# retinal-information-processing-lab/gaussian_processes

Hardware: AMD Instinct MI355X
Metric: GP fits/sec (kernel+chol+solve+grad loglik) at N=8192 d=256 (higher is better)
Workload: dtype f64; 1 GPU; N=8192 d=256 single cell f64, one M-step closure evaluation with 6 gradients (BASELINE configs[2], headline); N=8192, d=256, parallelism=independent units over 1 GPU(s), one process per GPU, no data-path collective

## Files before the change

### gaussian_processes_amd/_lib.py

```python
from __future__ import annotations

import ctypes
import os

from .build import lib_path

vp, i32, i64, f64 = ctypes.c_void_p, ctypes.c_int, ctypes.c_int64, ctypes.c_double
pd = ctypes.POINTER(ctypes.c_double)



class DevGemmArgs(ctypes.Structure):
    _fields_ = ([(n, vp) for n in ("A", "B", "C")] + [(n, i64) for n in ("lda", "ldb", "ldc", "sA", "sB", "sC")] +
                [("alpha", f64), ("beta", f64)] +
                [(n, vp) for n in ("sk_ws", "aux", "sumsq", "Ap", "Bp", "Cp", "auxp", "sumsqp")] +
                [(n, ctypes.c_int32) for n in ("M", "N", "K", "a_kmajor", "b_kmajor", "out_lower", "a_tri", "b_tri", "batch",
                                               "split_k", "tile", "walk", "epi", "nptr", "k_slabs")])


class DevGemmRoute(ctypes.Structure):
    _fields_ = [(n, ctypes.c_int32) for n in ("rc", "tile", "sk_first", "xcd", "stages", "half_occ", "edge", "epi",
                                              "sumsq_entries", "blocks", "pair", "slabs")]


_SIGS = {
    "gpfit_version": (i32, []),
    "gpfit_last_error": (ctypes.c_char_p, []),
    "gpfit_dgemm": (i32, [vp, i32, i32, i32, i32, i32, f64, vp, i64, vp, i64, f64, vp, i64, i32, i32, i32]),
    "gpfit_dgemm_ex": (i32, [vp, i32, i32, i32, i32, i32, f64, vp, i64, vp, i64, f64, vp, i64, i32, i32, i32, i32, i32]),
    "gpfit_ctx_create": (i32, [i32, i64, i64, i64, ctypes.POINTER(vp)]),
    "gpfit_ctx_destroy": (None, [vp]),
    "gpfit_check_limits": (i32, [pd, pd, pd]),
    "gpfit_localker_mask": (i32, [pd, i32, i32, vp, ctypes.POINTER(i64)]),
    "gpfit_localker": (i32, [vp, vp, pd, i32, i32, vp, i64, vp, vp]),
    "gpfit_acosker": (i32, [vp, vp, f64, vp, i64, i64, vp, i64, i64, i64, vp, i64, vp, vp, i64, vp]),
    "gpfit_acosker_pullback": (i32, [vp, vp, f64, vp, i64, i64, vp, i64, i64, i64, vp, i64, vp, i64, vp, vp, i64, pd]),
    "gpfit_acosker_diag": (i32, [vp, vp, f64, vp, i64, i64, i64, vp, i64, vp, vp, vp]),
# ... 83 lines not shown
```

### gaussian_processes_amd/csrc/api_dev.hip

```cpp
#include "gemm_core.h"
#include "context.h"
#include "gpfit_mi355x.h"

#include <cstring>

namespace gpfit {
namespace {

template <typename R>
int fill(const gpfit_dev_gemm_args& d, GemmArgsT<R>& g) {
  g = GemmArgsT<R>{};
  g.A = (const R*)d.A; g.B = (const R*)d.B; g.C = (R*)d.C;
  g.lda = d.lda; g.ldb = d.ldb; g.ldc = d.ldc;
  g.M = d.M; g.N = d.N; g.K = d.K;
  g.alpha = d.alpha; g.beta = d.beta;
  g.a_kmajor = d.a_kmajor; g.b_kmajor = d.b_kmajor;
  g.out_lower = d.out_lower; g.a_tri = d.a_tri; g.b_tri = d.b_tri;
  g.batch = d.batch > 0 ? d.batch : 1;
  g.sA = d.sA; g.sB = d.sB; g.sC = d.sC;
  g.split_k = d.split_k > 0 ? d.split_k : 1;
  g.k_slabs = d.k_slabs > 0 ? d.k_slabs : 0;
  g.tile = d.tile;
  g.reverse = d.walk & 15;
  g.half_occ = (d.walk >> 4) & 1;
  g.sk_ws = d.sk_ws;
  g.epi = d.epi;
  g.aux = (R*)d.aux;
  g.sumsq = d.sumsq;
  g.nptr = d.nptr;
  if (d.nptr < 0 || d.nptr > GEMM_MAXB) return d.nptr < 0 ? -3 : 0;
  for (int b = 0; b < d.nptr; ++b) {
    if (!d.Ap || !d.Bp || !d.Cp) return -3;
    g.Ap[b] = (const R*)d.Ap[b];
    g.Bp[b] = (const R*)d.Bp[b];
    g.Cp[b] = (R*)d.Cp[b];
    g.auxp[b] = d.auxp ? (R*)d.auxp[b] : nullptr;
    g.sumsqp[b] = d.sumsqp ? d.sumsqp[b] : nullptr;
  }
  return 0;
}

template <typename R>
int route(const gpfit_dev_gemm_args& d, const gpfit_dev_gemm_args* d2, gpfit_dev_gemm_route_t& o) {
  std::memset(&o, 0, sizeof(o));
  o.sk_first = -1;
  GemmArgsT<R> a, b;
  if (fill(d, a) != 0 || (d2 && fill(*d2, b) != 0)) return -3;
  GemmRoute r = d2 ? gemm_pair_shape(a, b) : gemm_route(a);
  long blocks = d2 ? r.tiles : -1;
  if (r.rc == 0 && r.sched == GEMM_STREAMK) {
    SkHostPlan plan;
    if (streamk_plan_host(a, r.sk_first, plan) != 0) r.stay_data_parallel();
    else blocks = plan.blocks;
  }
  if (r.rc == 0 && r.sched == GEMM_XCD) {
    std::vector<int> table;
    if (xcd_plan_host(a, table) != 0) return -3;
    r.gx = (int)table.size();
  }
  o.rc = r.rc; o.tile = r.tile; o.sk_first = r.sk_first; o.xcd = r.sched == GEMM_XCD; o.stages = r.stages;
  o.half_occ = r.half; o.edge = r.edge; o.epi = r.epi; o.sumsq_entries = r.sumsq_entries; o.slabs = r.slabs;
  o.pair = d2 && r.rc == 0;
  o.blocks = (int)std::min<long>(blocks >= 0 ? blocks : (long)r.gx * r.gy * r.gz, 0x7fffffffL);
  return 0;
}

template <typename R>
int64_t plan(const gpfit_dev_gemm_args& d, int kind, int32_t* out, int64_t cap) {
  GemmArgsT<R> a;
  if (fill(d, a) != 0 || a.M <= 0 || a.N <= 0) return -3;
  const GemmRoute r = gemm_route(a);
  if (r.rc != 0) return -3;
  if (kind == 1) {
    if (r.sched != GEMM_XCD) return -1;
    std::vector<int> table;
    if (xcd_plan_host(a, table) != 0) return -1;
// ... 112 lines not shown
```

### gaussian_processes_amd/csrc/common.h

```cpp
#pragma once
#include <hip/hip_runtime.h>
#include <stdint.h>
#include <stdio.h>
#include <string>

namespace gpfit {

constexpr double PI32 = 3.1415927410125732;

constexpr int TILE = 128;
constexpr int TRMV_ROWS = 128;
constexpr int KTILE = 16;

void set_error(const std::string& msg);

#define GP_HIP(expr)                                                                     \
  do {                                                                                   \
    hipError_t _e = (expr);                                                              \
    if (_e != hipSuccess) {                                                              \
      gpfit::set_error(std::string(#expr) + ": " + hipGetErrorString(_e));               \
      return -100;                                                                       \
    }                                                                                    \
  } while (0)

// ... 14 lines not shown
  R* C;
  int64_t lda, ldb, ldc;
  int M, N, K;
  double alpha, beta;
  int a_kmajor, b_kmajor;
  int out_lower;
  int a_tri, b_tri;
  int batch;
  int64_t sA, sB, sC;
  int split_k;
  int k_slabs;
  int tile;
  int reverse;
  int half_occ;
  void* sk_ws;
  int reserved;
  const int* sched;
  int epi;
  R* aux;
  double* sumsq;
  int nptr;
  const R* Ap[GEMM_MAXB];
  const R* Bp[GEMM_MAXB];
  R* Cp[GEMM_MAXB];
  R* auxp[GEMM_MAXB];
  double* sumsqp[GEMM_MAXB];
};
using GemmArgs = GemmArgsT<double>;

constexpr int SLAB_TILE = 64;
struct SlabPlan {
  int nt, ks, live;
  int full, rb;
  int items;
};
__host__ __device__ inline SlabPlan slab_plan(int M, int slabs) {
  SlabPlan p;
  p.nt = (M + SLAB_TILE - 1) / SLAB_TILE;
  p.ks = (p.nt + slabs - 1) / slabs;
  p.live = (p.nt + p.ks - 1) / p.ks;
  p.full = p.live + p.ks * (p.live * (p.live - 1) / 2);
// ... 28 lines not shown
enum { GEMM_DATA_PARALLEL = 0, GEMM_XCD = 1, GEMM_STREAMK = 2 };
struct GemmRoute {
  int rc;
  const char* error;
  int sched;
  int sk_first;
  int tile;
  int tiles, tiles_n;
  int stages;
  int edge;
  int half;
  int gx, gy, gz;
  int epi;
  int sumsq_entries;
  int slabs;
  void stay_data_parallel() { sched = GEMM_DATA_PARALLEL; sk_first = -1; gx = tiles; }
};
template <typename R> GemmRoute gemm_route(const GemmArgsT<R>& a);
template <typename R> int gemm_pick_tile(const GemmArgsT<R>& a);
template <typename R> int launch_gemm(const GemmArgsT<R>& a, const GemmRoute& r, hipStream_t s);
template <typename R> int launch_gemm(const GemmArgsT<R>& a, hipStream_t s) { return launch_gemm(a, gemm_route(a), s); }
template <typename R> int launch_gemm_streamk(const GemmArgsT<R>& a, const GemmRoute& r, hipStream_t s);
template <typename R> int launch_gemm_xcd(const GemmArgsT<R>& a, GemmRoute r, hipStream_t s);
template <typename R> int launch_gemm_plain(const GemmArgsT<R>& a, const GemmRoute& r, hipStream_t s);
template <typename R> GemmRoute gemm_pair_shape(const GemmArgsT<R>& a, const GemmArgsT<R>& b);
template <typename R> int launch_gemm_pair(const GemmArgsT<R>& a, const GemmArgsT<R>& b, const GemmRoute& h, hipStream_t s);

template <typename R>
struct GramArgsT {
  const R* XCt;
// ... 18 lines not shown
```

### gaussian_processes_amd/csrc/fit.hip

```cpp
#include "product.h"
#include "gemm_core.h"
#include "gpfit_mi355x.h"

#include <algorithm>
#include <chrono>
#include <cmath>
#include <cstdlib>
#include <cstring>
#include <limits>

namespace gpfit {

static thread_local gpfit_ctx* g_prof = nullptr;

static int walk(Walk which) {
  static int w[W_COUNT] = {3, 2, 1, 9, 9, 2, 2};
  static bool init = false;
  if (!init) {
    init = true;
    if (const char* e = getenv("GPFIT_WALKS")) {
      int v[W_COUNT];
      if (sscanf(e, "%d,%d,%d,%d,%d,%d,%d", &v[0], &v[1], &v[2], &v[3], &v[4], &v[5], &v[6]) == 7)
        for (int i = 0; i < W_COUNT; ++i) w[i] = v[i];
    }
// ... 126 lines not shown
  const int64_t slab = (int64_t)d.M * C.ld;
  bool any = false;
  for (int i = 0; i < cnt && !off; ++i)
    any = any || (partial[i] && std::min<int64_t>(splitk_for(d.M, d.N, d.K), partial_elems[i] / std::max<int64_t>(1, slab)) > 1);
  if (!any) return product(lane, d, alpha, a, b, into(C));
  for (int i = 0; i < cnt; ++i) {
    Operand<R> ai = a, bi = b;
    ai.m.cnt = bi.m.cnt = 1;
    ai.m.p[0] = a.m.p[i]; bi.m.p[0] = b.m.p[i];
    GP_TRY(gemm_splitk(lane, d, alpha, ai, bi, C.p[i], C.ld, partial[i], partial_elems[i]));
  }
  return 0;
}

static int fused_epilogues() {
  static const int v = getenv("GPFIT_FUSED_EPI") ? atoi(getenv("GPFIT_FUSED_EPI")) : 7;
  return v;
}

template <typename R>
int product(Lane lane, Dims d, double alpha, const Operand<R>& a, const Operand<R>& b, const Output<R>& c, int walk, Epilogue<R>* e) {
  const int cnt = c.m.cnt, epi = e ? e->which : 0;
  if (e) { e->carried = false; e->sumsq_entries = 0; }
  if (cnt <= 0) return 0;
  if (cnt > GEMM_MAXB) {
    set_error("product: more problems than a pointer batch holds");
    return -3;
  }
  GemmArgsT<R> g = product_args(lane, d, alpha, a, b, c, walk);
  static const bool no_batch = getenv("GPFIT_NO_BATCH") != nullptr;
  if (cnt == 1 || gemm_pick_tile(g) == TILE || no_batch) {
    auto problem = [&](int i, bool fused) {
      g.A = a.m.p[i]; g.B = b.m.p[i]; g.C = c.m.p[i];
      g.epi = fused ? epi : 0; g.aux = fused ? e->aux[i] : nullptr; g.sumsq = fused ? e->sumsq[i] : nullptr;
    };
    GemmRoute routes[GEMM_MAXB];
    bool fused = epi != 0;
    for (int i = 0; i < cnt && fused; ++i) {
      problem(i, true);
      routes[i] = gemm_route(g);
      fused = routes[i].epi != 0;
    }
    for (int i = 0; i < cnt; ++i) {
      problem(i, fused);
      GP_TRY(fused ? run_gemm(lane.s, g, routes[i]) : run_gemm(lane.s, g));
    }
    if (e) e->carried = fused;
    if (fused) e->sumsq_entries = routes[0].sumsq_entries;
    return 0;
  }
  g = batch_args(lane, d, alpha, a, b, c, walk, e);
  GemmRoute r = gemm_route(g);
  if (epi && r.epi == 0) {
    g.epi = 0;
    r = gemm_route(g);
  }
  if (e) { e->carried = g.epi != 0; e->sumsq_entries = r.sumsq_entries; }
  return run_gemm(lane.s, g, r);
}
template int product<double>(Lane, Dims, double, const Operand<double>&, const Operand<double>&, const Output<double>&, int,
                             Epilogue<double>*);
template int product<float>(Lane, Dims, double, const Operand<float>&, const Operand<float>&, const Output<float>&, int,
                            Epilogue<float>*);

template <typename R>
int potrf_lockstep(const CholBatchT<R>& B, int r0, int n, uint32_t need, Lane lane, uint32_t halves) {
  const int64_t ld = B.ld;
  const hipStream_t s = lane.s;
  const uint32_t all = (B.nb >= 32) ? 0xffffffffu : ((1u << B.nb) - 1u);
// ... 72 lines not shown
    GP_TRY(product(lane, {n2, n1, n2}, -1.0, plain(tril(blk(need, B.Li, r1, r1))), plain(blk(need, B.Tmp, r1, r0)),
                   into(blk(need, B.Li, r1, r0)), walk(W_MERGE)));
  }
  return 0;
}

template int potrf_lockstep<double>(const CholBatchT<double>&, int, int, uint32_t, Lane, uint32_t);
template int potrf_lockstep<float>(const CholBatchT<float>&, int, int, uint32_t, Lane, uint32_t);

template <typename R>
struct TwoSidedBufs { R* Q; const R* Li; R *W, *Z, *H; const R* L; int64_t ld; int min_split; };
template <typename R, typename P>
static Mat<P> ts_blk(int cnt, const TwoSidedBufs<R>* b, const int* r0, P* TwoSidedBufs<R>::*X, int dr, int dc) {
  return mats(cnt, b[0].ld, [&](int i) { const int o = r0 ? r0[i] : 0; return b[i].*X + (int64_t)(o + dr) * b[i].ld + o + dc; });
}
template <typename R>
static int dual_update_list(Lane lane, Dims d, double alpha, const Operand<R>& a, const Operand<R>& b, const Mat<R>& H,
                            const Mat<R>& Z, int wk) {
  const int cnt = H.cnt;
  const int64_t ld = H.ld;
  Epilogue<R> e{4};
  for (int i = 0; i < cnt; ++i) e.aux[i] = Z.p[i];
  bool fused = false;
  if (fused_epilogues() & 4) {
    GemmArgsT<R> g = product_args(lane, d, alpha, a, b, into(H), wk);
    g.epi = 4; g.aux = Z.p[0];
    static const bool no_batch = getenv("GPFIT_NO_BATCH") != nullptr;
    if (cnt > 1 && gemm_pick_tile(g) != TILE && !no_batch) { g.nptr = cnt; g.batch = cnt; }
    fused = gemm_route(g).epi != 0;
  }
  if (fused) {
    GP_TRY(product(lane, d, alpha, a, b, into(H), wk, &e));
    if (!e.carried) {
      set_error("two_sided: the dual-update epilogue was announced but not carried");
      return -100;
    }
    return 0;
  }
  for (int i = 0; i < cnt; ++i)
    GP_HIP(hipMemcpy2DAsync(H.p[i], (size_t)ld * sizeof(R), Z.p[i], (size_t)ld * sizeof(R), (size_t)d.N * sizeof(R), (size_t)d.M,
                            hipMemcpyDeviceToDevice, lane.s));
  GP_TRY(product(lane, d, alpha, a, b, into(H, 1.0), wk));
  for (int i = 0; i < cnt; ++i) GP_TRY(launch_axpby_block<R>(Z.p[i], ld, H.p[i], ld, d.M, d.N, 1.0, 1.0, lane.s));
  return 0;
}

template <typename R>
static int two_sided_list(Lane lane, int cnt, const TwoSidedBufs<R>* b, const int* r0, int n) {
  if (cnt <= 0) return 0;
  using TS = TwoSidedBufs<R>;
  auto blk = [&](auto X, int dr, int dc) { return ts_blk(cnt, b, r0, X, dr, dc); };
  const int k = n / TILE;
  if (n < b[0].min_split || k < 2) {
    static const int wbase_walk = getenv("GPFIT_WBASE_WALK") ? atoi(getenv("GPFIT_WBASE_WALK")) : 0;
    GP_TRY(product(lane, {n, n, n}, 1.0, trans(blk(&TS::Q, 0, 0)), plain(tril(blk(&TS::Li, 0, 0))), into(blk(&TS::Z, 0, 0)),
                   walk(W_RBASE)));
    return product(lane, {n, n, n}, 0.5, trans(tril(blk(&TS::Li, 0, 0))), plain(blk(&TS::Z, 0, 0)),
// ... 420 lines not shown
    Epilogue<R> ep{};
    for (int q = 0; q < cnt * cb && q < GEMM_MAXB; ++q) ep.sumsq[q] = cs[q / cb]->frob_part + ent + (q % cb) * e;
    GP_TRY(normed_product({nblk, nblk, nblk}, plain(tril(blk(&PJ::Li))), plain(tril(blk(&PJ::LV))), into_lower(blk(&PJ::T)),
                          walk(W_T), ask, ep, "a diagonal block of T"));
    ent += cb * e;
    return 0;
  };
  const int r_both[2] = {0, n1};
  if (n2 == n1 && 2 * cnt <= GEMM_MAXB) GP_TRY(diag_blocks(2, r_both, n1));
  else {
    GP_TRY(diag_blocks(1, r_both, n1));
    GP_TRY(diag_blocks(1, r_both + 1, n2));
  }
  {
    auto blk = [&](auto X, int64_t o) { return mats(cnt, ld, [&](int i) { return a[i].*X + o; }); };
    for (int i = 0; i < cnt; ++i)
      GP_HIP(hipMemcpy2DAsync(a[i].Z + o21, (size_t)ld * sizeof(R), a[i].LV + o21, (size_t)ld * sizeof(R), (size_t)n1 * sizeof(R),
                              (size_t)n2, hipMemcpyDeviceToDevice, s));
    GP_TRY(product(lane, {n2, n1, n1}, -1.0, plain(blk(&PJ::L, o21)), plain(tril(blk(&PJ::T, 0))), into(blk(&PJ::Z, o21), 1.0),
                   walk(W_TMP)));
    int e = asks_21();
    const bool ask = e > 0;
    if (!ask) e = (n2 / TILE) * (n1 / TILE);
    Epilogue<R> ep{};
    for (int i = 0; i < cnt; ++i) ep.sumsq[i] = cs[i]->frob_part + ent;
    GP_TRY(normed_product({n2, n1, n2}, plain(tril(blk(&PJ::Li, o21 + n1))), plain(blk(&PJ::Z, o21)), into(blk(&PJ::T, o21)),
                          walk(W_MERGE), ask, ep, "T21"));
    ent += e;
  }
  for (int i = 0; i < cnt; ++i) {
    if (any_fused) GP_TRY(launch_frob_finish(cs[i]->frob_part, ent, cs[i]->scal + S_TRACE, s));
    else GP_TRY(launch_frob_lower(a[i].T, ld, np, cs[i]->scal + S_TRACE, cs[i]->frob_part, s));
  }
  return 0;
}
// ... 10 lines not shown
    Epilogue<R> e{(fused_epilogues() & 2) ? 2 : 0};
    for (int i = 0; i < cnt; ++i) e.sumsq[i] = cs[i]->frob_part;
    GP_TRY(product(lane, {np, np, np}, 1.0, plain(tril(all(&PJ::Li, ld))), plain(tril(all(&PJ::LV, ld))), into_lower(all(&PJ::T, ld)),
                   walk(W_T), &e));
    for (int i = 0; i < cnt; ++i) {
      if (e.carried) GP_TRY(launch_frob_finish(cs[i]->frob_part, e.sumsq_entries, cs[i]->scal + S_TRACE, s));
      else GP_TRY(launch_frob_lower(a[i].T, ld, np, cs[i]->scal + S_TRACE, cs[i]->frob_part, s));
    }
  } else {
    GP_TRY(t_in_blocks<R>(lane, cnt, cs, a, np));
  }
  phase(4, s);
  if (!want_grad) return 0;
  {
    Epilogue<R> mirror{(fused_epilogues() & 1) ? 1 : 0};
    GP_TRY(product(lane, {np, np, np}, -1.0, plain(tril(all(&PJ::T, ld))), trans(tril(all(&PJ::T, ld))), into_lower(all(&PJ::W, ld)),
                   walk(W_Q), &mirror));
    for (int i = 0; i < cnt; ++i) {
      GP_TRY(launch_add_diag(a[i].W, ld, np, 1.0, s));
      if (!mirror.carried) GP_TRY(launch_symmetrize(a[i].W, ld, np, s));
    }
  }
  phase(5, s);
  {
    static const int ts_min = getenv("GPFIT_TS_MIN") ? atoi(getenv("GPFIT_TS_MIN")) : 4096;
    TwoSidedBufs<R> tb[GEMM_MAXB];
    for (int i = 0; i < cnt; ++i)
      tb[i] = TwoSidedBufs<R>{a[i].W, a[i].Li, a[i].T, a[i].Z, a[i].H, a[i].L, ld, ts_min > 0 ? ts_min : (1 << 30)};
    if (blocks) GP_TRY(two_sided_top<R>(lane, cnt, tb, np));
    else {
      int r0[GEMM_MAXB];
      for (int i = 0; i < cnt; ++i) r0[i] = 0;
      GP_TRY(two_sided_list<R>(lane, cnt, tb, r0, np));
    }
  }
// ... 52 lines not shown
  const bool blocks = top_in_blocks(np, sizeof(R));
  c->cur_n = n; c->cur_np = np; c->cur_d = d; c->cur_dp = dp;

  ++g_eval_count;
  const auto t_host0 = std::chrono::steady_clock::now();
  auto phase = [&](int i, hipStream_t st) {
    if (c->profile != 2) return;
    if (!c->phase_ev[i]) (void)hipEventCreate(&c->phase_ev[i]);
    (void)hipEventRecord(c->phase_ev[i], st);
  };
  c->phase_valid = false;
  phase(0, s);
  const Lane lane = main_lane(c, s);
  prof_begin(c);
  struct ProfGuard { gpfit_ctx* c; ~ProfGuard() { prof_end(c); } } prof_guard{c};
  GP_HIP(hipMemsetAsync(c->info, 0, 4 * sizeof(int), s));
  GP_HIP(hipMemcpyAsync(c->pix, c->pix_host, (size_t)d * sizeof(int), hipMemcpyHostToDevice, s));
  GP_HIP(hipMemsetAsync(RP(c->mpad), 0, (size_t)np * sizeof(R), s));
  GP_HIP(hipMemcpyAsync(RP(c->mpad), m, (size_t)n * sizeof(R), hipMemcpyDeviceToDevice, s));

  const bool reuse_V = (want_grad & 2) && c->lv_valid && c->lv_n == n && c->lv_bytes == (int)sizeof(R);
  const bool async_call = (want_grad & 4) != 0;
  const bool mixed_grad = (want_grad & 8) != 0 && sizeof(R) == 8 && (want_grad & 1);
  want_grad &= 1;
  static const int side_min_env = getenv("GPFIT_SIDE_MIN") ? atoi(getenv("GPFIT_SIDE_MIN")) : 1024;
  const int side_min = async_call ? 0 : side_min_env;
  if (!async_call) GP_TRY(ensure_side_stream(c));
  c->side_ev_next = 0;
  if (!reuse_V) {
    c->lv_valid = false; c->lv32_valid = false;
    GP_HIP(hipEventRecord(c->ev_fork, s));
    GP_HIP(hipStreamWaitEvent(c->aux, c->ev_fork, 0));
    GP_TRY(launch_pack_lower(V, ldv, n, RP(c->Vbuf), ld, np, c->aux));
    GP_HIP(hipEventRecord(c->ev_join, c->aux));
  }

  GP_TRY(build_kernel<R>(c, lane, th, d, dp, n_rows, n_cols, X, ldx, n, np, 0));
  GP_TRY(launch_moments(RP(c->Kvec), RP(c->q), RP(c->Cos), ld, V, ldv, m, r, n, A, lambda0, RP(c->lam_m), RP(c->lam_var), RP(c->fvec),
                        RP(c->wl), c->scal + S_RLAM, c->sumA_part, c->info + INFO_MOMENTS, s));
  phase(1, s);
  {
    CholBatchT<R> cb;
    cb.nb = reuse_V ? 1 : 2;
    cb.A[0] = RP(c->Kbuf); cb.L[0] = RP(c->Lbuf); cb.Li[0] = RP(c->Libuf); cb.Tmp[0] = RP(c->Tmp); cb.info[0] = c->info + INFO_K;
    cb.A[1] = RP(c->Vbuf); cb.L[1] = RP(c->LVbuf); cb.Li[1] = RP(c->LiVbuf); cb.Tmp[1] = RP(c->TmpV); cb.info[1] = c->info + INFO_V;
    cb.ld = ld; cb.ctx = c; cb.side_min = side_min;
    if (!reuse_V) GP_HIP(hipStreamWaitEvent(s, c->ev_join, 0));
    if (blocks) GP_TRY(potrf_lockstep<R>(cb, 0, np, 0u, lane, 1u));
    else GP_TRY(potrf_lockstep<R>(cb, 0, np, 1u, lane));
    if (!reuse_V) GP_TRY(launch_logdet(RP(c->LVbuf), ld, n, c->scal + S_LOGDET_V, s));
    phase(3, s);
  }
  GP_TRY(launch_logdet(RP(c->Lbuf), ld, n, c->scal + S_LOGDET_K, s));
  GP_TRY(solve_mean<R>(c, np, blocks, s));

  phase(2, s);
  if (mixed_grad) {
    PostJoin<float> pf;
    GP_TRY(demote_for_mixed(c, reuse_V, np, dp, blocks, s, &pf));
    GP_TRY(post_join_list<float>(lane, 1, &c, &pf, &th, n, np, &d, &dp, n_rows, n_cols, want_grad, blocks, phase));
  } else {
    const PostJoin<R> pj = post_join_args<R>(c);
    GP_TRY(post_join_list<R>(lane, 1, &c, &pj, &th, n, np, &d, &dp, n_rows, n_cols, want_grad, blocks, phase));
  }

  if (lam_m_out) GP_HIP(hipMemcpyAsync(lam_m_out, RP(c->lam_m), (size_t)n * sizeof(R), hipMemcpyDeviceToDevice, s));
  if (lam_var_out) GP_HIP(hipMemcpyAsync(lam_var_out, RP(c->lam_var), (size_t)n * sizeof(R), hipMemcpyDeviceToDevice, s));
  if (f_out) GP_HIP(hipMemcpyAsync(f_out, RP(c->fvec), (size_t)n * sizeof(R), hipMemcpyDeviceToDevice, s));
  GP_HIP(hipMemcpyAsync(c->scal_host, c->scal, 64 * sizeof(double), hipMemcpyDeviceToHost, s));
  GP_HIP(hipMemcpyAsync(c->info_host, c->info, 4 * sizeof(int), hipMemcpyDeviceToHost, s));
  phase(7, s);
  c->phase_valid = (c->profile == 2 && want_grad && !reuse_V);
  c->last_enqueue_ms = std::chrono::duration<double, std::milli>(std::chrono::steady_clock::now() - t_host0).count();
  set_pending(c, s, A, lambda0, th.sigma0, n, np, d, want_grad, (int)sizeof(R), false);
  if (async_call) return 0;
  return fit_eval_finish(c, out_host);
}

template <typename R>
static int fit_eval_batch_impl(gpfit_ctx* const* cs, int nu, void* stream, const double* theta6, const double* lower,
                               const double* upper, int n_rows, int n_cols, const R* const* X, int64_t ldx, int64_t N,
                               const R* const* r, const R* const* m, const R* const* V, int64_t ldv, const double* logA,
                               const double* lambda0, int want_grad, double* out_host, int* rc_out) {
  auto RP = ws_as<R>;
  if (!cs || nu <= 0 || 2 * nu > GEMM_MAXB || !theta6 || !X || !r || !m || !V || !logA || !lambda0 || !out_host || !rc_out ||
      N <= 0) {
    set_error("gpfit_fit_eval_batch: bad argument (1 .. 16 units per call)");
    return -3;
  }
// ... 709 lines not shown
```

### gaussian_processes_amd/csrc/gemm.hip

```cpp
#include "gemm_core.h"

#include <algorithm>
#include <cstdlib>
#include <mutex>
#include <set>
#include <utility>

namespace gpfit {

template <typename R, bool A_KMAJOR, bool B_KMAJOR, bool EDGE, int T, int NS>
__device__ __forceinline__ bool gemm_tile_compute(const GemmArgsT<R>& p, int tiles_n, int ntiles, R* smem,
                                                  typename Real<R>::acc_t (&acc)[T / 32][T / 32], int& ti, int& tj,
                                                  int& row0, int& col0, R*& C) {
  constexpr int KT = Real<R>::KT;

  int slab = 0, slab_tiles = 0;
  const bool slabbed = (T == SLAB_TILE) && p.k_slabs > 0;
  if (slabbed) {
    const SlabPlan sp = slab_plan(p.M, p.k_slabs);
    slab_item(sp, (int)blockIdx.x / tiles_n, ti, slab);
    tj = (int)blockIdx.x % tiles_n;
    slab_tiles = sp.ks;
  } else if (p.sched != nullptr) {
    const int e = p.sched[blockIdx.x];
// ... 46 lines not shown
template <typename R, bool A_KMAJOR, bool B_KMAJOR, bool EDGE, int T, int NS, int EPI = 0>
__device__ __forceinline__ void gemm_tile_body(const GemmArgsT<R>& p, int tiles_n, int ntiles, R* smem) {
  typename Real<R>::acc_t acc[T / 32][T / 32];
  int ti, tj, row0, col0;
  R* C;
  if (!gemm_tile_compute<R, A_KMAJOR, B_KMAJOR, EDGE, T, NS>(p, tiles_n, ntiles, smem, acc, ti, tj, row0, col0, C)) return;

  const R alpha = (R)p.alpha, beta = (p.split_k > 1 || (T == SLAB_TILE && p.k_slabs > 0)) ? (R)0 : (R)p.beta;
  const int64_t ldc = p.ldc;
  const int M = p.M, N = p.N;
  if constexpr (EPI != 0) {
    constexpr int epi = EPI;
    R* __restrict__ D = p.nptr > 0 ? p.auxp[blockIdx.y] : p.aux;
    double* __restrict__ sumsq = p.nptr > 0 ? p.sumsqp[blockIdx.y] : p.sumsq;
    double ss = 0.0;
    for_each_acc<R, T>(acc, row0, col0, [&](int row, int col, R v) {
      if (EDGE && !(row < M && col < N)) return;
      R o = alpha * v;
      R* c = C + (int64_t)row * ldc + col;
      if (epi & 4) {
        R* dd = D + (int64_t)row * ldc + col;
        const R d0 = *dd;
        o += d0;
        *dd = o + d0;
      } else if (beta != (R)0) {
        o += beta * (*c);
      }
      if (epi & 1) {
        if (row >= col) *c = o;
        if (row > col) C[(int64_t)col * ldc + row] = o;
      } else {
        *c = o;
      }
      if (epi & 2) ss += (double)o * (double)o;
    });
    if (epi & 2) {
#pragma unroll
      for (int o = 32; o > 0; o >>= 1) ss += __shfl_down(ss, o);
      double* red = reinterpret_cast<double*>(smem);
      __syncthreads();
      if ((threadIdx.x & 63) == 0) red[threadIdx.x >> 6] = ss;
      __syncthreads();
      if (threadIdx.x == 0)
        sumsq[p.out_lower ? (int64_t)ti * (ti + 1) / 2 + tj : (int64_t)ti * tiles_n + tj] = (red[0] + red[1]) + (red[2] + red[3]);
    }
    return;
  }
  if (beta == (R)0) {
    for_each_acc<R, T>(acc, row0, col0, [&](int row, int col, R v) {
      if (!EDGE || (row < M && col < N)) C[(int64_t)row * ldc + col] = alpha * v;
    });
  } else {
    for_each_acc<R, T>(acc, row0, col0, [&](int row, int col, R v) {
      if (!EDGE || (row < M && col < N)) {
        R* c = C + (int64_t)row * ldc + col;
        *c = alpha * v + beta * (*c);
      }
    });
  }
}

template <typename R, bool A_KMAJOR, bool B_KMAJOR, bool EDGE, int T, int NS = 2>
__global__ __launch_bounds__(GEMM_THREADS, (T == 128 || NS > 2 ? 2 : 4)) void gemm_mfma_kernel(GemmArgsT<R> p,
                                                                                               int tiles_n,
                                                                                               int ntiles) {
  __shared__ __attribute__((aligned(16))) R smem[2 * NS * Real<R>::KT * T];
  gemm_tile_body<R, A_KMAJOR, B_KMAJOR, EDGE, T, NS>(p, tiles_n, ntiles, smem);
}

#ifdef GPFIT_CLOCK_STAMPS
__device__ long long g_gemm_clock[2][4096][2];
// ... 102 lines not shown
      (a.tile == 0 || a.tile == TILE)) {
    static const long xcd_min = getenv("GPFIT_XCD_MIN_TILES") ? atol(getenv("GPFIT_XCD_MIN_TILES")) : 1536;
    const long tm = a.M / TILE, tn = a.N / TILE, ntiles = a.out_lower ? tm * (tm + 1) / 2 : tm * tn;
    if ((a.reverse & 8) && !(a.out_lower && a.M != a.N) && tm < 32768 && tn < 32768 && ntiles >= xcd_min) r.sched = GEMM_XCD;
    else if ((r.sk_first = streamk_first_tile(a, ntiles)) >= 0) r.sched = GEMM_STREAMK;
  }

  if (a.epi) {
    bool ok = a.split_k <= 1 && a.k_slabs <= 0 && !strided && T == TILE && !(a.M % T) && !(a.N % T) && !a.a_kmajor && !a.half_occ;
    if ((a.epi & 1) && (!a.out_lower || a.M != a.N)) ok = false;
    if ((a.epi & 4) && a.nptr <= 0 && a.aux == nullptr) ok = false;
    if (!((a.epi == 2 && a.b_kmajor) || (a.epi == 1 && !a.b_kmajor) || (a.epi == 4 && a.b_kmajor))) ok = false;
    if (r.sched == GEMM_STREAMK && !(r.sk_first == 0 && a.out_lower && a.M == a.N && a.epi == 2 && a.sumsq != nullptr)) ok = false;
    if (!ok) return refuse("launch_gemm: this launch cannot carry a fused epilogue (gemm_route says so beforehand)");
  }
  constexpr int EPC = 16 / (int)sizeof(R);
  if (a.K % ktile_of<R>() != 0 || (a.lda % EPC) || (a.ldb % EPC))
    return refuse("launch_gemm: K must be a multiple of the K step and lda, ldb multiples of 16 bytes");
  if (a.out_lower && a.M != a.N) return refuse("launch_gemm: out_lower needs a square output");
  if (a.nptr > 0 && (a.nptr > GEMM_MAXB || a.sched || a.split_k > 1))
    return refuse("launch_gemm: a pointer batch holds at most GEMM_MAXB plain problems");
  if (a.k_slabs > 0 &&
      (a.a_tri != 2 || a.b_tri || a.out_lower || a.M != a.K || (a.M % SLAB_TILE) || a.split_k > 1 || a.sched ||
       a.half_occ || strided || (a.tile != 0 && a.tile != SLAB_TILE)))
    return refuse("launch_gemm: k_slabs needs an upper triangular square op(A) on whole 64-tiles and a plain launch");

  r.epi = a.epi;
  if (a.epi & 2) r.sumsq_entries = (r.sched == GEMM_STREAMK ? 33 : 1) * r.tiles;
  r.gx = r.sched == GEMM_XCD ? 0 : (r.sched == GEMM_STREAMK ? r.sk_first : r.tiles);
  if (a.k_slabs > 0) {
    const SlabPlan sp = slab_plan(a.M, a.k_slabs);
    r.gx = sp.items * r.tiles_n;
    r.slabs = sp.live;
  }
  r.gy = a.nptr > 0 ? a.nptr : std::max(a.batch, 1);
  r.gz = a.split_k > 1 ? a.split_k : 1;
  r.stages = gemm_stages(T, r.edge, (long)r.gx * r.gy * r.gz);
  r.half = T == TILE && a.half_occ;
  return r;
}
template GemmRoute gemm_route<double>(const GemmArgsT<double>&);
template GemmRoute gemm_route<float>(const GemmArgsT<float>&);
// ... 81 lines not shown
};

template <typename R, int T, int NS>
__global__ __launch_bounds__(GEMM_THREADS, (NS > 2 ? 2 : 4)) void gemm_pair_kernel(GemmPairT<R> q) {
  __shared__ __attribute__((aligned(16))) R smem[2 * NS * Real<R>::KT * T];
  const int w = blockIdx.z;
  const GemmArgsT<R>& p = q.g[w];
  if ((int)blockIdx.x >= q.tiles[w] || (int)blockIdx.y >= p.batch) return;
  if (p.b_kmajor) gemm_tile_body<R, false, true, false, T, NS>(p, q.tiles_n[w], q.tiles[w], smem);
  else gemm_tile_body<R, false, false, false, T, NS>(p, q.tiles_n[w], q.tiles[w], smem);
}

template <typename R>
static GemmRoute pair_member_route(const GemmArgsT<R>& a) {
  const GemmRoute none{};
  if (a.nptr <= 0 || a.epi || a.k_slabs > 0 || a.half_occ || a.a_kmajor || (a.M % 64) || (a.N % 64)) return none;
  const GemmRoute r = gemm_route(a);
  return (r.rc == 0 && !r.edge && (r.tile == 32 || r.tile == 64)) ? r : none;
}

template <typename R>
GemmRoute gemm_pair_shape(const GemmArgsT<R>& a, const GemmArgsT<R>& b) {
  static const bool off = getenv("GPFIT_NO_PAIR") != nullptr;
  static const bool no64 = getenv("GPFIT_NO_PAIR64") != nullptr;
  GemmRoute h{};
  h.sk_first = -1;
  const GemmRoute ra = pair_member_route(a), rb = pair_member_route(b);
  if (off || ra.tile == 0 || ra.tile != rb.tile || (no64 && ra.tile == 64)) {
    h.rc = -3;
    h.error = "launch_gemm_pair: the two problems cannot share a launch (gemm_pair_shape says so beforehand)";
    return h;
// ... 55 lines not shown
```

### gaussian_processes_amd/csrc/product.h

```cpp
#pragma once
#include "context.h"
#include <type_traits>

namespace gpfit {

enum Tri { Dense = 0, Lower = 1, Upper = 2 };
struct Dims { int M, N, K; };

template <typename R> struct Mat { int cnt; int64_t ld; Tri tri; R* p[GEMM_MAXB]; };
template <typename R>
Mat<R> mat(R* p, int64_t ld) {
  Mat<R> m{};
  m.cnt = 1; m.ld = ld; m.p[0] = p;
  return m;
}
template <typename F>
auto mats(int cnt, int64_t ld, F&& at) {
  Mat<std::remove_pointer_t<decltype(at(0))>> m{};
  m.cnt = cnt; m.ld = ld;
  for (int i = 0; i < cnt && i < GEMM_MAXB; ++i) m.p[i] = at(i);
  return m;
}
template <typename R> Mat<R> tril(Mat<R> m) { m.tri = Lower; return m; }
template <typename R> Mat<R> triu(Mat<R> m) { m.tri = Upper; return m; }

template <typename R> struct Operand { Mat<const R> m; bool t; };
template <typename R> Operand<R> plain(const Mat<const R>& m) { return {m, false}; }
template <typename R> Operand<R> trans(const Mat<const R>& m) { return {m, true}; }
template <typename R> Operand<R> plain(const Mat<R>& m) {
  Operand<R> o{{m.cnt, m.ld, m.tri, {}}, false};
  for (int i = 0; i < m.cnt && i < GEMM_MAXB; ++i) o.m.p[i] = m.p[i];
  return o;
}
template <typename R> Operand<R> trans(const Mat<R>& m) { Operand<R> o = plain(m); o.t = true; return o; }

template <typename R> struct Output { Mat<R> m; bool lower; double beta; };
template <typename R> Output<R> into(const Mat<R>& m, double beta = 0.0) { return {m, false, beta}; }
template <typename R> Output<R> into_lower(const Mat<R>& m, double beta = 0.0) { return {m, true, beta}; }

template <typename R> struct Epilogue { int which; R* aux[GEMM_MAXB]; double* sumsq[GEMM_MAXB]; bool carried; int sumsq_entries; };

template <typename R>
GemmArgsT<R> product_args(Lane lane, Dims d, double alpha, const Operand<R>& a, const Operand<R>& b, const Output<R>& c,
                          int walk = 0) {
  auto tri = [](const Operand<R>& o) { return (o.t && o.m.tri != Dense) ? (int)Lower + (int)Upper - (int)o.m.tri : (int)o.m.tri; };
  GemmArgsT<R> g{};
  g.A = a.m.p[0]; g.B = b.m.p[0]; g.C = c.m.p[0];
  g.lda = a.m.ld; g.ldb = b.m.ld; g.ldc = c.m.ld;
  g.M = d.M; g.N = d.N; g.K = d.K;
  g.alpha = alpha; g.beta = c.beta;
  g.a_kmajor = a.t ? 1 : 0; g.b_kmajor = b.t ? 0 : 1;
  g.out_lower = c.lower ? 1 : 0; g.a_tri = tri(a); g.b_tri = tri(b);
  g.batch = 1; g.split_k = 1; g.reverse = walk; g.sk_ws = lane.sk_ws;
  return g;
}
template <typename R>
GemmArgsT<R> batch_args(Lane lane, Dims d, double alpha, const Operand<R>& a, const Operand<R>& b, const Output<R>& c,
                        int walk = 0, const Epilogue<R>* e = nullptr) {
  GemmArgsT<R> g = product_args(lane, d, alpha, a, b, c, walk);
  g.nptr = g.batch = c.m.cnt;
  for (int i = 0; i < c.m.cnt; ++i) {
    g.Ap[i] = a.m.p[i]; g.Bp[i] = b.m.p[i]; g.Cp[i] = c.m.p[i];
    g.auxp[i] = e ? e->aux[i] : nullptr; g.sumsqp[i] = e ? e->sumsq[i] : nullptr;
  }
  g.epi = e ? e->which : 0;
  return g;
}

template <typename R> int run_gemm(hipStream_t s, const GemmArgsT<R>& g, const GemmRoute& r);
template <typename R> int run_gemm(hipStream_t s, const GemmArgsT<R>& g) { return run_gemm(s, g, gemm_route(g)); }
template <typename R>
int product(Lane lane, Dims d, double alpha, const Operand<R>& a, const Operand<R>& b, const Output<R>& c, int walk = 0,
            Epilogue<R>* e = nullptr);

}
```

### include/gpfit_mi355x.h

```cpp
#ifndef GPFIT_MI355X_H
#define GPFIT_MI355X_H

#include <stdint.h>

#ifdef __cplusplus
extern "C" {
#endif

#define GPFIT_VERSION 100

int gpfit_version(void);
const char* gpfit_last_error(void);

int gpfit_dgemm(void* stream, int a_kmajor, int b_kmajor, int M, int N, int K, double alpha,
                const double* A, int64_t lda, const double* B, int64_t ldb, double beta, double* C,
                int64_t ldc, int out_lower, int a_tri, int b_tri);
int gpfit_dgemm_ex(void* stream, int a_kmajor, int b_kmajor, int M, int N, int K, double alpha,
                   const double* A, int64_t lda, const double* B, int64_t ldb, double beta, double* C,
                   int64_t ldc, int out_lower, int a_tri, int b_tri, int walk, int tile);

typedef struct gpfit_ctx gpfit_ctx;
int gpfit_ctx_create(int device, int64_t n_max, int64_t d_max, int64_t d_full_max, gpfit_ctx** out);
void gpfit_ctx_destroy(gpfit_ctx* ctx);

// ... 131 lines not shown
  double* sumsq;
  const void* const* Ap;
  const void* const* Bp;
  void* const* Cp;
  void* const* auxp;
  double* const* sumsqp;
  int32_t M, N, K;
  int32_t a_kmajor, b_kmajor, out_lower, a_tri, b_tri;
  int32_t batch;
  int32_t split_k;
  int32_t tile;
  int32_t walk;
  int32_t epi;
  int32_t nptr;
  int32_t k_slabs;
} gpfit_dev_gemm_args;

typedef struct gpfit_dev_gemm_route_t {
  int32_t rc;
  int32_t tile;
  int32_t sk_first;
  int32_t xcd;
  int32_t stages;
  int32_t half_occ;
  int32_t edge;
  int32_t epi;
  int32_t sumsq_entries;
  int32_t blocks;
  int32_t pair;
  int32_t slabs;
} gpfit_dev_gemm_route_t;

int gpfit_dev_gemm_route(int is_f32, const gpfit_dev_gemm_args* args, const gpfit_dev_gemm_args* pair_args,
                         gpfit_dev_gemm_route_t* out);
int64_t gpfit_dev_gemm_plan(int is_f32, const gpfit_dev_gemm_args* args, int kind, int32_t* out, int64_t cap);
int gpfit_dev_gemm(void* stream, int is_f32, const gpfit_dev_gemm_args* args, const gpfit_dev_gemm_args* pair_args);
int gpfit_dev_ctx_copy(gpfit_ctx* ctx, const char* name, int64_t offset, void* dev, int64_t bytes, int to_ctx);
int gpfit_dev_ctx_fill(gpfit_ctx* ctx, const char* name, int byte);

#ifdef __cplusplus
}
#endif
#endif
```

Before: 36.55 fits/s.

## Fuse copies, diag add and logdets into GEMM epilogues and grouped launches

Adds a second-source beta input (Cin) to the GEMM epilogue so the device-to-device copy before each C += A·B update is folded into the product. Folds the W diagonal add into the mirror epilogue and limits mirroring to tiles past a threshold. Also pairs the two logdet launches into one, and replaces the per-call memset/memcpy prep and the host readback with grouped prepare/collect kernels plus an event record. This trims launch count and memory traffic, at the cost of more epilogue branching, a wider args struct and reliance on route fallbacks.

```diff
diff --git a/gaussian_processes_amd/_lib.py b/gaussian_processes_amd/_lib.py
--- a/gaussian_processes_amd/_lib.py
+++ b/gaussian_processes_amd/_lib.py
@@ -15,12 +15,13 @@
                 [("alpha", f64), ("beta", f64)] +
                 [(n, vp) for n in ("sk_ws", "aux", "sumsq", "Ap", "Bp", "Cp", "auxp", "sumsqp")] +
                 [(n, ctypes.c_int32) for n in ("M", "N", "K", "a_kmajor", "b_kmajor", "out_lower", "a_tri", "b_tri", "batch",
-                                               "split_k", "tile", "walk", "epi", "nptr", "k_slabs")])
+                                               "split_k", "tile", "walk", "epi", "nptr", "k_slabs", "mirror_from")] +
+                [("diag", f64), ("Cin", vp), ("Cinp", vp)])
 
 
 class DevGemmRoute(ctypes.Structure):
     _fields_ = [(n, ctypes.c_int32) for n in ("rc", "tile", "sk_first", "xcd", "stages", "half_occ", "edge", "epi",
-                                              "sumsq_entries", "blocks", "pair", "slabs")]
+                                              "sumsq_entries", "blocks", "pair", "slabs", "cin")]
 
 
 _SIGS = {
diff --git a/gaussian_processes_amd/csrc/api_dev.hip b/gaussian_processes_amd/csrc/api_dev.hip
--- a/gaussian_processes_amd/csrc/api_dev.hip
+++ b/gaussian_processes_amd/csrc/api_dev.hip
@@ -27,6 +27,8 @@
   g.epi = d.epi;
   g.aux = (R*)d.aux;
   g.sumsq = d.sumsq;
+  g.mirror_from = d.mirror_from; g.diag = d.diag;
+  g.Cin = (const R*)d.Cin;
   g.nptr = d.nptr;
   if (d.nptr < 0 || d.nptr > GEMM_MAXB) return d.nptr < 0 ? -3 : 0;
   for (int b = 0; b < d.nptr; ++b) {
@@ -36,6 +38,7 @@
     g.Cp[b] = (R*)d.Cp[b];
     g.auxp[b] = d.auxp ? (R*)d.auxp[b] : nullptr;
     g.sumsqp[b] = d.sumsqp ? d.sumsqp[b] : nullptr;
+    g.Cinp[b] = d.Cinp ? (const R*)d.Cinp[b] : nullptr;
   }
   return 0;
 }
@@ -60,6 +63,7 @@
   }
   o.rc = r.rc; o.tile = r.tile; o.sk_first = r.sk_first; o.xcd = r.sched == GEMM_XCD; o.stages = r.stages;
   o.half_occ = r.half; o.edge = r.edge; o.epi = r.epi; o.sumsq_entries = r.sumsq_entries; o.slabs = r.slabs;
+  o.cin = r.cin;
   o.pair = d2 && r.rc == 0;
   o.blocks = (int)std::min<long>(blocks >= 0 ? blocks : (long)r.gx * r.gy * r.gz, 0x7fffffffL);
   return 0;
diff --git a/gaussian_processes_amd/csrc/common.h b/gaussian_processes_amd/csrc/common.h
--- a/gaussian_processes_amd/csrc/common.h
+++ b/gaussian_processes_amd/csrc/common.h
@@ -52,17 +52,21 @@
   int reverse;
   int half_occ;
   void* sk_ws;
-  int reserved;
+  int mirror_from;
   const int* sched;
   int epi;
   R* aux;
   double* sumsq;
+  double diag;
+  const R* Cin;
   int nptr;
   const R* Ap[GEMM_MAXB];
   const R* Bp[GEMM_MAXB];
   R* Cp[GEMM_MAXB];
   R* auxp[GEMM_MAXB];
   double* sumsqp[GEMM_MAXB];
+  const R* Cinp[GEMM_MAXB];
+  bool has_cin() const { return nptr > 0 ? Cinp[0] != nullptr : Cin != nullptr; }
 };
 using GemmArgs = GemmArgsT<double>;
 
@@ -121,6 +125,7 @@
   int epi;
   int sumsq_entries;
   int slabs;
+  int cin;
   void stay_data_parallel() { sched = GEMM_DATA_PARALLEL; sk_first = -1; gx = tiles; }
 };
 template <typename R> GemmRoute gemm_route(const GemmArgsT<R>& a);
diff --git a/gaussian_processes_amd/csrc/fit.hip b/gaussian_processes_amd/csrc/fit.hip
--- a/gaussian_processes_amd/csrc/fit.hip
+++ b/gaussian_processes_amd/csrc/fit.hip
@@ -164,7 +164,7 @@
 }
 
 static int fused_epilogues() {
-  static const int v = getenv("GPFIT_FUSED_EPI") ? atoi(getenv("GPFIT_FUSED_EPI")) : 7;
+  static const int v = getenv("GPFIT_FUSED_EPI") ? atoi(getenv("GPFIT_FUSED_EPI")) : 15;
   return v;
 }
 
@@ -181,8 +181,9 @@
   static const bool no_batch = getenv("GPFIT_NO_BATCH") != nullptr;
   if (cnt == 1 || gemm_pick_tile(g) == TILE || no_batch) {
     auto problem = [&](int i, bool fused) {
-      g.A = a.m.p[i]; g.B = b.m.p[i]; g.C = c.m.p[i];
+      g.A = a.m.p[i]; g.B = b.m.p[i]; g.C = c.m.p[i]; g.Cin = c.src[i];
       g.epi = fused ? epi : 0; g.aux = fused ? e->aux[i] : nullptr; g.sumsq = fused ? e->sumsq[i] : nullptr;
+      g.mirror_from = fused ? e->mirror_from : 0; g.diag = fused ? e->diag : 0.0;
     };
     GemmRoute routes[GEMM_MAXB];
     bool fused = epi != 0;
@@ -202,7 +203,7 @@
   g = batch_args(lane, d, alpha, a, b, c, walk, e);
   GemmRoute r = gemm_route(g);
   if (epi && r.epi == 0) {
-    g.epi = 0;
+    g.epi = 0; g.mirror_from = 0; g.diag = 0.0;
     r = gemm_route(g);
   }
   if (e) { e->carried = g.epi != 0; e->sumsq_entries = r.sumsq_entries; }
@@ -305,6 +306,26 @@
 static Mat<P> ts_blk(int cnt, const TwoSidedBufs<R>* b, const int* r0, P* TwoSidedBufs<R>::*X, int dr, int dc) {
   return mats(cnt, b[0].ld, [&](int i) { const int o = r0 ? r0[i] : 0; return b[i].*X + (int64_t)(o + dr) * b[i].ld + o + dc; });
 }
+template <typename R, typename S>
+static int product_plus(Lane lane, Dims d, double alpha, const Operand<R>& a, const Operand<R>& b, const Mat<R>& C, const Mat<S>& src,
+                        int wk) {
+  const int cnt = C.cnt;
+  const int64_t ld = C.ld;
+  bool direct = false;
+  if (fused_epilogues() & 8) {
+    static const bool no_batch = getenv("GPFIT_NO_BATCH") != nullptr;
+    GemmArgsT<R> g = product_args(lane, d, alpha, a, b, into_from(C, src, 1.0), wk);
+    if (cnt > 1 && gemm_pick_tile(g) != TILE && !no_batch) g = batch_args(lane, d, alpha, a, b, into_from(C, src, 1.0), wk);
+    const GemmRoute r = gemm_route(g);
+    direct = r.rc == 0 && r.cin;
+  }
+  if (direct) return product(lane, d, alpha, a, b, into_from(C, src, 1.0), wk);
+  for (int i = 0; i < cnt; ++i)
+    GP_HIP(hipMemcpy2DAsync(C.p[i], (size_t)ld * sizeof(R), src.p[i], (size_t)ld * sizeof(R), (size_t)d.N * sizeof(R), (size_t)d.M,
+                            hipMemcpyDeviceToDevice, lane.s));
+  return product(lane, d, alpha, a, b, into(C, 1.0), wk);
+}
+
 template <typename R>
 static int dual_update_list(Lane lane, Dims d, double alpha, const Operand<R>& a, const Operand<R>& b, const Mat<R>& H,
                             const Mat<R>& Z, int wk) {
@@ -328,10 +349,7 @@
     }
     return 0;
   }
-  for (int i = 0; i < cnt; ++i)
-    GP_HIP(hipMemcpy2DAsync(H.p[i], (size_t)ld * sizeof(R), Z.p[i], (size_t)ld * sizeof(R), (size_t)d.N * sizeof(R), (size_t)d.M,
-                            hipMemcpyDeviceToDevice, lane.s));
-  GP_TRY(product(lane, d, alpha, a, b, into(H, 1.0), wk));
+  GP_TRY(product_plus(lane, d, alpha, a, b, H, Z, wk));
   for (int i = 0; i < cnt; ++i) GP_TRY(launch_axpby_block<R>(Z.p[i], ld, H.p[i], ld, d.M, d.N, 1.0, 1.0, lane.s));
   return 0;
 }
@@ -782,11 +800,8 @@
   }
   {
     auto blk = [&](auto X, int64_t o) { return mats(cnt, ld, [&](int i) { return a[i].*X + o; }); };
-    for (int i = 0; i < cnt; ++i)
-      GP_HIP(hipMemcpy2DAsync(a[i].Z + o21, (size_t)ld * sizeof(R), a[i].LV + o21, (size_t)ld * sizeof(R), (size_t)n1 * sizeof(R),
-                              (size_t)n2, hipMemcpyDeviceToDevice, s));
-    GP_TRY(product(lane, {n2, n1, n1}, -1.0, plain(blk(&PJ::L, o21)), plain(tril(blk(&PJ::T, 0))), into(blk(&PJ::Z, o21), 1.0),
-                   walk(W_TMP)));
+    GP_TRY(product_plus(lane, {n2, n1, n1}, -1.0, plain(blk(&PJ::L, o21)), plain(tril(blk(&PJ::T, 0))), blk(&PJ::Z, o21),
+                        blk(&PJ::LV, o21), walk(W_TMP)));
     int e = asks_21();
     const bool ask = e > 0;
     if (!ask) e = (n2 / TILE) * (n1 / TILE);
@@ -827,11 +842,14 @@
   if (!want_grad) return 0;
   {
     Epilogue<R> mirror{(fused_epilogues() & 1) ? 1 : 0};
+    const int n1 = ((np / TILE + 1) / 2) * TILE;
+    mirror.mirror_from = blocks ? n1 / TILE : 0;
+    mirror.diag = 1.0;
     GP_TRY(product(lane, {np, np, np}, -1.0, plain(tril(all(&PJ::T, ld))), trans(tril(all(&PJ::T, ld))), into_lower(all(&PJ::W, ld)),
                    walk(W_Q), &mirror));
-    for (int i = 0; i < cnt; ++i) {
+    for (int i = 0; i < cnt && !mirror.carried; ++i) {
       GP_TRY(launch_add_diag(a[i].W, ld, np, 1.0, s));
-      if (!mirror.carried) GP_TRY(launch_symmetrize(a[i].W, ld, np, s));
+      GP_TRY(launch_symmetrize(a[i].W, ld, np, s));
     }
   }
   phase(5, s);
@@ -914,10 +932,13 @@
   const Lane lane = main_lane(c, s);
   prof_begin(c);
   struct ProfGuard { gpfit_ctx* c; ~ProfGuard() { prof_end(c); } } prof_guard{c};
-  GP_HIP(hipMemsetAsync(c->info, 0, 4 * sizeof(int), s));
-  GP_HIP(hipMemcpyAsync(c->pix, c->pix_host, (size_t)d * sizeof(int), hipMemcpyHostToDevice, s));
-  GP_HIP(hipMemsetAsync(RP(c->mpad), 0, (size_t)np * sizeof(R), s));
-  GP_HIP(hipMemcpyAsync(RP(c->mpad), m, (size_t)n * sizeof(R), hipMemcpyDeviceToDevice, s));
+  {
+    GroupPrepT<R> gp{};
+    gp.n_units = 1; gp.n = n; gp.np = np;
+    gp.pix_host[0] = c->pix_host; gp.pix[0] = c->pix; gp.d[0] = d; gp.info[0] = c->info;
+    gp.m[0] = m; gp.mpad[0] = RP(c->mpad);
+    GP_TRY(launch_group_prepare(gp, s));
+  }
 
   const bool reuse_V = (want_grad & 2) && c->lv_valid && c->lv_n == n && c->lv_bytes == (int)sizeof(R);
   const bool async_call = (want_grad & 4) != 0;
@@ -948,10 +969,10 @@
     if (!reuse_V) GP_HIP(hipStreamWaitEvent(s, c->ev_join, 0));
     if (blocks) GP_TRY(potrf_lockstep<R>(cb, 0, np, 0u, lane, 1u));
     else GP_TRY(potrf_lockstep<R>(cb, 0, np, 1u, lane));
-    if (!reuse_V) GP_TRY(launch_logdet(RP(c->LVbuf), ld, n, c->scal + S_LOGDET_V, s));
     phase(3, s);
   }
-  GP_TRY(launch_logdet(RP(c->Lbuf), ld, n, c->scal + S_LOGDET_K, s));
+  if (!reuse_V) GP_TRY(launch_logdet_pair(RP(c->Lbuf), c->scal + S_LOGDET_K, RP(c->LVbuf), c->scal + S_LOGDET_V, ld, n, s));
+  else GP_TRY(launch_logdet(RP(c->Lbuf), ld, n, c->scal + S_LOGDET_K, s));
   GP_TRY(solve_mean<R>(c, np, blocks, s));
 
   phase(2, s);
@@ -967,12 +988,18 @@
   if (lam_m_out) GP_HIP(hipMemcpyAsync(lam_m_out, RP(c->lam_m), (size_t)n * sizeof(R), hipMemcpyDeviceToDevice, s));
   if (lam_var_out) GP_HIP(hipMemcpyAsync(lam_var_out, RP(c->lam_var), (size_t)n * sizeof(R), hipMemcpyDeviceToDevice, s));
   if (f_out) GP_HIP(hipMemcpyAsync(f_out, RP(c->fvec), (size_t)n * sizeof(R), hipMemcpyDeviceToDevice, s));
-  GP_HIP(hipMemcpyAsync(c->scal_host, c->scal, 64 * sizeof(double), hipMemcpyDeviceToHost, s));
-  GP_HIP(hipMemcpyAsync(c->info_host, c->info, 4 * sizeof(int), hipMemcpyDeviceToHost, s));
+  {
+    GroupCollectT gc{};
+    gc.n_units = 1;
+    gc.scal[0] = c->scal; gc.info[0] = c->info; gc.scal_host[0] = c->scal_host; gc.info_host[0] = c->info_host;
+    GP_TRY(launch_group_collect(gc, s));
+  }
   phase(7, s);
+  if (!c->pend.done) GP_HIP(hipEventCreateWithFlags(&c->pend.done, hipEventDisableTiming));
+  GP_HIP(hipEventRecord(c->pend.done, s));
   c->phase_valid = (c->profile == 2 && want_grad && !reuse_V);
   c->last_enqueue_ms = std::chrono::duration<double, std::milli>(std::chrono::steady_clock::now() - t_host0).count();
-  set_pending(c, s, A, lambda0, th.sigma0, n, np, d, want_grad, (int)sizeof(R), false);
+  set_pending(c, s, A, lambda0, th.sigma0, n, np, d, want_grad, (int)sizeof(R), true);
   if (async_call) return 0;
   return fit_eval_finish(c, out_host);
 }
diff --git a/gaussian_processes_amd/csrc/gemm.hip b/gaussian_processes_amd/csrc/gemm.hip
--- a/gaussian_processes_amd/csrc/gemm.hip
+++ b/gaussian_processes_amd/csrc/gemm.hip
@@ -84,6 +84,9 @@
     R* __restrict__ D = p.nptr > 0 ? p.auxp[blockIdx.y] : p.aux;
     double* __restrict__ sumsq = p.nptr > 0 ? p.sumsqp[blockIdx.y] : p.sumsq;
     double ss = 0.0;
+    const bool mirrored = (epi & 1) && (tj >= p.mirror_from || ti == tj);
+    const R diag = (R)p.diag;
+    const bool on_diag = (epi & 1) && ti == tj && diag != (R)0;
     for_each_acc<R, T>(acc, row0, col0, [&](int row, int col, R v) {
       if (EDGE && !(row < M && col < N)) return;
       R o = alpha * v;
@@ -97,8 +100,9 @@
         o += beta * (*c);
       }
       if (epi & 1) {
+        if (on_diag && row == col) o += diag;
         if (row >= col) *c = o;
-        if (row > col) C[(int64_t)col * ldc + row] = o;
+        if (mirrored && row > col) C[(int64_t)col * ldc + row] = o;
       } else {
         *c = o;
       }
@@ -121,10 +125,12 @@
       if (!EDGE || (row < M && col < N)) C[(int64_t)row * ldc + col] = alpha * v;
     });
   } else {
+    const R* Cin = p.nptr > 0 ? p.Cinp[blockIdx.y] : p.Cin;
+    if (Cin == nullptr) Cin = C;
     for_each_acc<R, T>(acc, row0, col0, [&](int row, int col, R v) {
       if (!EDGE || (row < M && col < N)) {
-        R* c = C + (int64_t)row * ldc + col;
-        *c = alpha * v + beta * (*c);
+        const int64_t at = (int64_t)row * ldc + col;
+        C[at] = alpha * v + beta * Cin[at];
       }
     });
   }
@@ -257,6 +263,8 @@
     if (r.sched == GEMM_STREAMK && !(r.sk_first == 0 && a.out_lower && a.M == a.N && a.epi == 2 && a.sumsq != nullptr)) ok = false;
     if (!ok) return refuse("launch_gemm: this launch cannot carry a fused epilogue (gemm_route says so beforehand)");
   }
+  if (a.has_cin() && (r.sched == GEMM_STREAMK || a.split_k > 1 || a.k_slabs > 0 || a.epi || strided))
+    return refuse("launch_gemm: this launch cannot read its beta term from a second source (gemm_route says so beforehand)");
   constexpr int EPC = 16 / (int)sizeof(R);
   if (a.K % ktile_of<R>() != 0 || (a.lda % EPC) || (a.ldb % EPC))
     return refuse("launch_gemm: K must be a multiple of the K step and lda, ldb multiples of 16 bytes");
@@ -269,6 +277,7 @@
     return refuse("launch_gemm: k_slabs needs an upper triangular square op(A) on whole 64-tiles and a plain launch");
 
   r.epi = a.epi;
+  r.cin = a.has_cin() ? 1 : 0;
   if (a.epi & 2) r.sumsq_entries = (r.sched == GEMM_STREAMK ? 33 : 1) * r.tiles;
   r.gx = r.sched == GEMM_XCD ? 0 : (r.sched == GEMM_STREAMK ? r.sk_first : r.tiles);
   if (a.k_slabs > 0) {
@@ -380,7 +389,7 @@
 template <typename R>
 static GemmRoute pair_member_route(const GemmArgsT<R>& a) {
   const GemmRoute none{};
-  if (a.nptr <= 0 || a.epi || a.k_slabs > 0 || a.half_occ || a.a_kmajor || (a.M % 64) || (a.N % 64)) return none;
+  if (a.nptr <= 0 || a.epi || a.has_cin() || a.k_slabs > 0 || a.half_occ || a.a_kmajor || (a.M % 64) || (a.N % 64)) return none;
   const GemmRoute r = gemm_route(a);
   return (r.rc == 0 && !r.edge && (r.tile == 32 || r.tile == 64)) ? r : none;
 }
diff --git a/gaussian_processes_amd/csrc/product.h b/gaussian_processes_amd/csrc/product.h
--- a/gaussian_processes_amd/csrc/product.h
+++ b/gaussian_processes_amd/csrc/product.h
@@ -34,18 +34,25 @@
 }
 template <typename R> Operand<R> trans(const Mat<R>& m) { Operand<R> o = plain(m); o.t = true; return o; }
 
-template <typename R> struct Output { Mat<R> m; bool lower; double beta; };
-template <typename R> Output<R> into(const Mat<R>& m, double beta = 0.0) { return {m, false, beta}; }
-template <typename R> Output<R> into_lower(const Mat<R>& m, double beta = 0.0) { return {m, true, beta}; }
+template <typename R> struct Output { Mat<R> m; bool lower; double beta; const R* src[GEMM_MAXB]; };
+template <typename R> Output<R> into(const Mat<R>& m, double beta = 0.0) { return {m, false, beta, {}}; }
+template <typename R> Output<R> into_lower(const Mat<R>& m, double beta = 0.0) { return {m, true, beta, {}}; }
+template <typename R, typename S> Output<R> into_from(const Mat<R>& m, const Mat<S>& src, double beta) {
+  Output<R> o = into(m, beta);
+  for (int i = 0; i < m.cnt && i < GEMM_MAXB; ++i) o.src[i] = src.p[i];
+  return o;
+}
 
-template <typename R> struct Epilogue { int which; R* aux[GEMM_MAXB]; double* sumsq[GEMM_MAXB]; bool carried; int sumsq_entries; };
+template <typename R> struct Epilogue {
+  int which; R* aux[GEMM_MAXB]; double* sumsq[GEMM_MAXB]; bool carried; int sumsq_entries; int mirror_from; double diag;
+};
 
 template <typename R>
 GemmArgsT<R> product_args(Lane lane, Dims d, double alpha, const Operand<R>& a, const Operand<R>& b, const Output<R>& c,
                           int walk = 0) {
   auto tri = [](const Operand<R>& o) { return (o.t && o.m.tri != Dense) ? (int)Lower + (int)Upper - (int)o.m.tri : (int)o.m.tri; };
   GemmArgsT<R> g{};
-  g.A = a.m.p[0]; g.B = b.m.p[0]; g.C = c.m.p[0];
+  g.A = a.m.p[0]; g.B = b.m.p[0]; g.C = c.m.p[0]; g.Cin = c.src[0];
   g.lda = a.m.ld; g.ldb = b.m.ld; g.ldc = c.m.ld;
   g.M = d.M; g.N = d.N; g.K = d.K;
   g.alpha = alpha; g.beta = c.beta;
@@ -60,10 +67,11 @@
   GemmArgsT<R> g = product_args(lane, d, alpha, a, b, c, walk);
   g.nptr = g.batch = c.m.cnt;
   for (int i = 0; i < c.m.cnt; ++i) {
-    g.Ap[i] = a.m.p[i]; g.Bp[i] = b.m.p[i]; g.Cp[i] = c.m.p[i];
+    g.Ap[i] = a.m.p[i]; g.Bp[i] = b.m.p[i]; g.Cp[i] = c.m.p[i]; g.Cinp[i] = c.src[i];
     g.auxp[i] = e ? e->aux[i] : nullptr; g.sumsqp[i] = e ? e->sumsq[i] : nullptr;
   }
   g.epi = e ? e->which : 0;
+  g.mirror_from = e ? e->mirror_from : 0; g.diag = e ? e->diag : 0.0;
   return g;
 }
 
diff --git a/include/gpfit_mi355x.h b/include/gpfit_mi355x.h
--- a/include/gpfit_mi355x.h
+++ b/include/gpfit_mi355x.h
@@ -169,6 +169,10 @@
   int32_t epi;
   int32_t nptr;
   int32_t k_slabs;
+  int32_t mirror_from;
+  double diag;
+  const void* Cin;
+  const void* const* Cinp;
 } gpfit_dev_gemm_args;
 
 typedef struct gpfit_dev_gemm_route_t {
@@ -184,6 +188,7 @@
   int32_t blocks;
   int32_t pair;
   int32_t slabs;
+  int32_t cin;
 } gpfit_dev_gemm_route_t;
 
 int gpfit_dev_gemm_route(int is_f32, const gpfit_dev_gemm_args* args, const gpfit_dev_gemm_args* pair_args,
```

Result: no change. 36.68 fits/s (median of 6 runs) (+0.4%).
